# carltonyfakhry/geneticsCRE

Measured on AMD Instinct MI355X. Metric: path_x_permutation_scores_per_sec, higher is better.
Workload: dtype u32

## Files before the change

### geneticscre_amd/api.py

```python
from __future__ import annotations

import ctypes
import functools
import os
from dataclasses import dataclass
from typing import Dict, Optional, Tuple

import numpy as np

from . import build as _build

_LIB = None

GCRE_OK, GCRE_ERR_ASSERT, GCRE_ERR_RANGE, GCRE_ERR_DEVICE, GCRE_ERR_ARG = 0, -1, -2, -3, -4
EXPECTED_ABI = 4


class GcreError(RuntimeError):
    pass


class gcre_result(ctypes.Structure):
    _fields_ = [("n", ctypes.c_int32), ("scores", ctypes.POINTER(ctypes.c_double)),
                ("src", ctypes.POINTER(ctypes.c_int32)), ("trg", ctypes.POINTER(ctypes.c_int32)),
# ... 119 lines not shown
    "gcre_generate_weighted_masks", "gcre_weighted_thresholds", "gcre_weighted_launches",
    "gcre_score_sets_sequential_weighted",
    "gcre_score_sets_prefix_sequential", "gcre_score_sets_dose_sequential", "gcre_seq_prefix_launches",
    "gcre_set_overlap", "gcre_overlap_launches",
    "gcre_clump_sets", "gcre_clump_launches",
    "gcre_set_patient_counts", "gcre_patient_launches",
    "gcre_patient_burden", "gcre_burden_launches",
    "gcre_gene_tally_create", "gcre_join_set_tally", "gcre_process_paths_set_tally", "gcre_gene_tally_read",
    "gcre_gene_tally_free",
    "gcre_exceed_create", "gcre_join_set_exceed", "gcre_process_paths_set_exceed", "gcre_exceed_read",
    "gcre_exceed_reset", "gcre_exceed_free",
    "gcre_exceed_keep_perm_counts", "gcre_exceed_read_perm_counts",
    "gcre_exceed_stepdown", "gcre_stepdown_launches",
    "gcre_hits_create", "gcre_join_set_hits", "gcre_process_paths_set_hits", "gcre_hits_count", "gcre_hits_read",
    "gcre_hits_reset", "gcre_hits_free", "gcre_hits_launches",
    "gcre_test_range_union", "gcre_test_expand",
]


def lib_path() -> str:
    return _build.LIB


def load_library():
    global _LIB
    if _LIB is not None:
        return _LIB
    path = os.environ.get("GCRE_LIB") or _build.build()
    try:
        lib = ctypes.CDLL(path)
    except OSError as e:
# ... 56 lines not shown
    lib.gcre_resolve_count_locs.argtypes = [P, I64, P, P, P, I64, P, P]
    lib.gcre_build_levels.argtypes = [ctypes.c_int32, P, P, P, I64, ctypes.POINTER(gcre_levels)]
    lib.gcre_levels_free.argtypes = [ctypes.POINTER(gcre_levels)]
    lib.gcre_levels_free.restype = None
    lib.gcre_values_table.argtypes = [I, I, P]
    lib.gcre_values_table_exact_order.argtypes = [I, I]
    lib.gcre_rccl_selftest.argtypes = [I, ctypes.c_char_p, ctypes.c_size_t]
    lib.gcre_rccl_collectives.restype = ctypes.c_int64
    lib.gcre_generate_perm_masks.argtypes = [V, ctypes.c_uint64, P, I]
    lib.gcre_mix64.restype = ctypes.c_uint64
    lib.gcre_mix64.argtypes = [ctypes.c_uint64]
    lib.gcre_get_perm_mask.argtypes = [V, I, P]
    if hasattr(lib, "gcre_test_expand"):
        lib.gcre_test_range_union.argtypes = [V, P, I64, P, I64, P, P, P, I64, I, I, I, P, P, P]
        lib.gcre_test_expand.argtypes = [V, P, P, I64, P, I64, I, I, I64, I64, P, P]
    lib.gcre_uids_set_reduced.argtypes = [V, V, P, I64]
    lib.gcre_set_perm_window.argtypes = [V, I, I]
    lib.gcre_plan_perm_window.argtypes = [V, P, I]
    lib.gcre_set_inspect_cache.argtypes = [V, I]
    lib.gcre_drop_inspections.argtypes = [V, I]
    _LIB = lib
    return lib


def _ptr(a: Optional[np.ndarray]):
    return None if a is None else a.ctypes.data_as(ctypes.c_void_p)


_V = _P = ctypes.c_void_p
_I, _I32, _I64 = ctypes.c_int, ctypes.c_int32, ctypes.c_int64
# ... 1149 lines not shown
        piece = np.zeros(1, dtype=np.int32)
        self._check(self._lib.gcre_test_range_union(self._h, _ptr(p1), len(p1), _ptr(pz), len(pz), _ptr(zindex), _ptr(loc), _ptr(cnt),
                                                    len(loc), S, wp, method, _ptr(u), _ptr(bad), _ptr(piece)))
        return u, int(bad[0]), int(piece[0])

    def test_expand(self, path_idx, location, signs, path_length: int, method: int, first: int, count: int):
        path_idx = np.ascontiguousarray(path_idx, dtype=np.int64)
        location = np.ascontiguousarray(location, dtype=np.int64)
        signs = np.ascontiguousarray(signs, dtype=np.int32)
        row0 = np.full(max(count, 1), 0xffffffff, dtype=np.uint32)
        row1 = np.full(max(count, 1), 0xffffffff, dtype=np.uint32)
        self._check(self._lib.gcre_test_expand(self._h, _ptr(path_idx), _ptr(location), len(location), _ptr(signs), len(signs),
                                               int(path_length), int(method), int(first), int(count), _ptr(row0), _ptr(row1)))
        return row0[:count], row1[:count]

    def create_path_set(self, size: int) -> PathSet:
        return PathSet(self, self._lib.gcre_pathset_zeros(self._h, int(size)))

    def load(self, data) -> PathSet:
        d = np.ascontiguousarray(data, dtype=np.int32)
        ncol = d.shape[1] if d.ndim == 2 else 0
        return PathSet(self, self._lib.gcre_pathset_from_dense(self._h, _ptr(d), d.shape[0], ncol, 0))

    def from_words(self, rows) -> PathSet:
        r = np.ascontiguousarray(rows, dtype=np.uint64).reshape(-1, self.vlen)
        return PathSet(self, self._lib.gcre_pathset_from_words(self._h, _ptr(r), r.shape[0]))

    def join(self, uids, paths0: PathSet, paths1: PathSet, paths_res: Optional[PathSet] = None,
             shard: Optional[Tuple[int, int]] = None, d_null_out: int = 0,
             keep: Optional[Tuple[int, int]] = None, keep_mode: int = 1, exchange=None, exchanges: int = 0,
# ... 471 lines not shown
```

### geneticscre_amd/csrc/gcre_host.h

```cpp
#pragma once
#include "../../include/gcre_hip.h"
#include "gcre_kernels.h"
#include "gcre_pipeline.h"

#include <algorithm>
#include <array>
#include <atomic>
#include <chrono>
#include <cmath>
#include <cstdio>
#include <cstdlib>
#include <cstring>
#include <limits>
#include <memory>
#include <mutex>
#include <condition_variable>
#include <string>
#include <unordered_map>
#include <thread>
#include <functional>
#include <deque>
#include <vector>

using namespace gcre;
// ... 243 lines not shown
  int64_t strata_launches = 0;
  int64_t weighted_launches = 0;

  uint64_t* d_case_mask = nullptr;
  uint32_t* d_masks = nullptr;
  float* d_t32 = nullptr;
  double* d_dvt = nullptr;
  double* d_dmax = nullptr;
  double* d_dmaxn = nullptr;
  uint32_t* d_null = nullptr;
  uint32_t* d_mt = nullptr;
  bool mt_stale = false;
  int ieq_batch = 0;
  int ie_quad = 1;
  int ie_flagq = 1;
  int ie_zwide = 0;
  int ie_warm_items = 4;
  int ie_warm_div = 4096;
  int ie_warm_cap_div = 8;
  int exchange_tail = 0;
  int ie_warm_segs = 1024;
  int ie_small_join_tiles = 8;
  int ie_batch = 2;
  uint32_t* d_queue = nullptr;
  uint32_t* d_max_tot = nullptr;
  uint32_t* d_ladder = nullptr;
  uint32_t g00_rows = 0xffffffffu;
  int null_kernel = 0;
  int sparse_waves_per_cu = 32;
  int ie_prune = 1;
// ... 48 lines not shown
};

struct gcre_pathset {
  gcre_ctx* ctx;
  int64_t nrows;
  uint64_t* d_rows;
  uint64_t id = 0;
  mutable uint64_t version = 0;
  mutable gcre_recipe* rec = nullptr;
  mutable uint64_t* d_loff = nullptr;
  mutable uint32_t* d_lidx = nullptr;
  mutable std::vector<uint64_t> h_loff;
  mutable uint32_t max_bits = 0;
  mutable bool max_known = false;
  mutable int one_sided = -1;
  mutable uint32_t* d_planes = nullptr;
  mutable int plane_groups = 0;
  mutable size_t planes_bytes = 0;
  mutable uint64_t planes_epoch = 0;
  mutable bool planes_valid = false;
  mutable int64_t planes_lo = 0, planes_hi = 0;
  mutable bool planes_wanted = false;
};

struct gcre_uids {
  gcre_ctx* ctx;
  int path_length;
  int64_t n_uids;
  int64_t n_signs;
  int64_t total;
// ... 116 lines not shown
```

### geneticscre_amd/csrc/gcre_host.hip

```cpp
#include "gcre_host.h"

namespace {

thread_local std::string g_create_error;

inline bool poison_fresh_planes() {
  static const bool on = std::getenv("GCRE_POISON") != nullptr && std::atoi(std::getenv("GCRE_POISON")) != 0;
  return on;
}
inline void poison_planes(void* p, size_t bytes) {
  if (!poison_fresh_planes() || !p) return;
  (void)hipDeviceSynchronize();
  (void)hipMemset(p, 0x5A, bytes);
  (void)hipDeviceSynchronize();
}

inline size_t tri(size_t t) { return t * (t + 1) / 2; }

template <typename Pred>
void pack_bits_host(const int32_t* data, int64_t nrow, int ncol, bool col_major, uint64_t* out, size_t stride, Pred pred) {
  const int W = (ncol + 63) / 64;
  if (nrow <= 0 || W <= 0) return;
  unsigned T = std::min<unsigned>(16u, std::max(1u, std::thread::hardware_concurrency()));
  if (const char* e = std::getenv("GCRE_PACK_THREADS")) T = (unsigned)std::max(1, std::atoi(e));
// ... 164 lines not shown
        for (size_t k = 1; k < c->plane_pool.size(); k++)
          if (c->plane_pool[k].bytes < c->plane_pool[small].bytes) small = k;
        (void)hipFree(c->plane_pool[small].p);
        c->plane_pool.erase(c->plane_pool.begin() + (long)small);
      }
    } else {
      (void)hipFree(ps->d_planes);
    }
  }
  ps->d_planes = nullptr;
  ps->planes_bytes = 0;
  ps->plane_groups = 0;
  ps->planes_valid = false;
}

void drop_lists(const gcre_pathset* ps) {
  if (ps->d_loff) (void)hipFree(ps->d_loff);
  if (ps->d_lidx) (void)hipFree(ps->d_lidx);
  ps->d_loff = nullptr;
  ps->d_lidx = nullptr;
  ps->h_loff.clear();
  ps->max_bits = 0;
  ps->max_known = false;
  ps->one_sided = -1;
  drop_planes(ps);
}

int ensure_lists(gcre_ctx* c, const gcre_pathset* ps) {
  if (ps->d_loff) return GCRE_OK;
  HostTimer ht("ensure_lists");
  const Geometry& g = c->g;
// ... 28 lines not shown
  ps->h_loff = std::move(off);
  ps->max_bits = longest;
  ps->max_known = true;
  return GCRE_OK;
}

bool one_sided(const gcre_pathset* ps) {
  if (!ps->d_loff || ps->h_loff.size() != (size_t)ps->nrows * 2 + 1) return false;
  if (ps->one_sided < 0) {
    int yes = 1;
    for (int64_t r = 0; r < ps->nrows && yes; r++)
      if (ps->h_loff[(size_t)2 * r + 1] > ps->h_loff[(size_t)2 * r] && ps->h_loff[(size_t)2 * r + 2] > ps->h_loff[(size_t)2 * r + 1]) yes = 0;
    ps->one_sided = yes;
  }
  return ps->one_sided == 1;
}

uint32_t row_max(const gcre_ctx* c, const gcre_pathset* ps) {
  return ps->max_known ? ps->max_bits : (uint32_t)(64 * c->g.Wp);
}

int plane_groups_for(uint32_t max_count) {
  int bits = 1;
  while (bits < 16 && (max_count >> bits) != 0) bits++;
  return std::max(2, (bits + 3) / 4);
}

bool planes_cover(const gcre_ctx* c, const gcre_pathset* ps, int64_t lo, int64_t hi) {
  return ps->d_planes && ps->planes_valid && ps->planes_epoch == c->mask_epoch && (hi <= lo || (ps->planes_lo <= lo && hi <= ps->planes_hi));
}
// ... 1432 lines not shown
    sa.excess = R.hinted ? R.exbuf->p : nullptr;
    sa.range_of = R.hinted ? u.d_range_of : nullptr;
    sa.bad = R.flagblk + kFlagHintBroken;
    sa.ie_bias = 8;
    sa.ie_rule = g.method == 1 ? 1 : 0;
    sa.rowz = C.rowz;
    sa.linfo = C.linfo;
    sa.lover = C.lover;
    sa.slot = C.slot;
    sa.over = C.over;
    sa.over_cap = (uint32_t)std::min<size_t>(C.over_cap - 16, 0xfffffff0u);
    if (rcp && !C.hit) HIP_TRY(c, hipMemcpyAsync(rcp->row0.p + cb, b.row0.p, (size_t)n * 4, hipMemcpyDeviceToDevice, st));
    sa.ov_count = R.flagblk + kFlagOverReserved;
    sa.zoff = (uint32_t)(64 * g.Wp) << 8;
    if (g.method == 2 && one_sided(R.red)) sa.lz_off = R.red->d_loff;
    if (!C.hit) HIP_TRY(c, launch_stats_ie(sa, g.method, st));
    if (rcp && !C.hit)
      HIP_TRY(c, hipMemcpyAsync(rcp->tot.p + (size_t)cb * g.method, b.tot.p, nl * 4, hipMemcpyDeviceToDevice, st));
  } else if (!C.hit) {
    HIP_TRY(c, launch_stats(sa, g.method, st));
  }
  if (!C.hit) {
    HIP_TRY(c, hipEventRecord(e1, st));
    if (R.mode != kInspect) HIP_TRY(c, hipEventRecord(c->ev_insp_main, st));
    R.ev_stats->emplace_back(e0, e1);
    if (ci) {
      ci->inspected = true;
      ci->with_lists = C.use_ie;
      ci->in_recipe = C.use_ie && rcp != nullptr;
    }
// ... 739 lines not shown
  if (const char* e = std::getenv("GCRE_NULL_BLOCKS_PER_CU")) c->null_blocks_per_cu = std::max(1, std::atoi(e));
  if (const char* e = std::getenv("GCRE_NULL_KERNEL"))
    c->null_kernel = !std::strcmp(e, "dense") ? 1 : !std::strcmp(e, "sparse") ? 2 : !std::strcmp(e, "ie") ? 3 : 0;
  if (const char* e = std::getenv("GCRE_IE_PRUNE")) c->ie_prune = std::atoi(e) != 0;
  if (const char* e = std::getenv("GCRE_EXCHANGE_TAIL")) c->exchange_tail = std::min(std::max(std::atoi(e), -1), 64);
  if (const char* e = std::getenv("GCRE_IE_WARM")) c->ie_warm_segs = std::min(std::max(std::atoi(e), 0), 1 << 20);
  if (const char* e = std::getenv("GCRE_IE_WARM_ITEMS")) c->ie_warm_items = std::min(std::max(std::atoi(e), 1), 64);
  if (const char* e = std::getenv("GCRE_IE_WARM_DIV")) c->ie_warm_div = std::min(std::max(std::atoi(e), 1), 1 << 30);
  if (const char* e = std::getenv("GCRE_IE_WARM_CAP_DIV")) c->ie_warm_cap_div = std::min(std::max(std::atoi(e), 1), 1 << 30);
  if (const char* e = std::getenv("GCRE_IE_SJT")) c->ie_small_join_tiles = std::atoi(e);
  if (const char* e = std::getenv("GCRE_IE_BATCH")) c->ie_batch = std::min(std::max(std::atoi(e), 1), 4096);
  if (const char* e = std::getenv("GCRE_IEQ_BATCH")) c->ieq_batch = std::max(0, std::atoi(e));
  if (const char* e = std::getenv("GCRE_IE_QUAD")) c->ie_quad = std::min(std::max(std::atoi(e), 0), 2);
  if (const char* e = std::getenv("GCRE_IE_FLAGQ")) c->ie_flagq = std::atoi(e) != 0;
  if (const char* e = std::getenv("GCRE_IE_ZWIDE")) c->ie_zwide = std::atoi(e) != 0;
  if (const char* e = std::getenv("GCRE_PLANES_OUT_MAX_MB")) c->planes_out_max = (size_t)std::max(0ll, std::atoll(e)) << 20;
  if (const char* e = std::getenv("GCRE_SPARSE_WAVES_PER_CU")) c->sparse_waves_per_cu = std::max(1, std::atoi(e));

  bool ok = hipStreamCreateWithFlags(&c->stream, hipStreamNonBlocking) == hipSuccess;
  ok = ok && hipStreamCreateWithFlags(&c->sel_stream, hipStreamNonBlocking) == hipSuccess;
  ok = ok && hipStreamCreateWithFlags(&c->insp_stream, hipStreamNonBlocking) == hipSuccess;
  ok = ok && hipStreamCreateWithFlags(&c->rec_stream, hipStreamNonBlocking) == hipSuccess;
  ok = ok && hipEventCreateWithFlags(&c->ev_rec_in, hipEventDisableTiming) == hipSuccess;
  ok = ok && hipEventCreateWithFlags(&c->ev_rec_done, hipEventDisableTiming) == hipSuccess;
  if (const char* e = std::getenv("GCRE_REC_STREAM")) c->rec_async = std::atoi(e) != 0;
  ok = ok && hipEventCreateWithFlags(&c->ev_insp_done, hipEventDisableTiming) == hipSuccess;
  ok = ok && hipEventCreateWithFlags(&c->ev_insp_main, hipEventDisableTiming) == hipSuccess;
  ok = ok && hipEventCreateWithFlags(&c->ev_tail, hipEventDisableTiming) == hipSuccess;
  if (const char* e = std::getenv("GCRE_AHEAD")) c->ahead_on = std::atoi(e) != 0;
  ok = ok && hipEventCreateWithFlags(&c->ev_sel, hipEventDisableTiming) == hipSuccess;
// ... 362 lines not shown
  hipError_t e = dpi.upload(path_idx, (size_t)n_uids + 1, st);
  if (e == hipSuccess) e = dloc.upload(location, (size_t)n_uids, st);
  if (e == hipSuccess) e = dsg.upload(signs, (size_t)n_signs, st);
  if (e == hipSuccess) e = d0.reserve((size_t)count);
  if (e == hipSuccess) e = d1.reserve((size_t)count);
  if (e == hipSuccess) e = launch_expand(dpi.p, dloc.p, n_uids, dsg.p, path_length, method, first, count, d0.p, d1.p, st);
  if (e == hipSuccess) e = hipMemcpyAsync(row0, d0.p, (size_t)count * 4, hipMemcpyDeviceToHost, st);
  if (e == hipSuccess) e = hipMemcpyAsync(row1, d1.p, (size_t)count * 4, hipMemcpyDeviceToHost, st);
  if (e == hipSuccess) e = hipStreamSynchronize(st);
  for (void* p : {(void*)dpi.p, (void*)dloc.p, (void*)dsg.p, (void*)d0.p, (void*)d1.p})
    if (p) (void)hipFree(p);
  if (e != hipSuccess) return fail(c, GCRE_ERR_DEVICE, std::string("gcre_test_expand: ") + hipGetErrorString(e));
  return GCRE_OK;
}

gcre_pathset* gcre_pathset_zeros(gcre_ctx* c, int64_t nrows) {
  if (!c) return nullptr;
  (void)hipSetDevice(c->device);
  return new_pathset(c, nrows, true);
}

gcre_pathset* gcre_pathset_from_dense(gcre_ctx* c, const int32_t* data, int64_t nrow, int ncol, int col_major) {
  if (!c) return nullptr;
  (void)hipSetDevice(c->device);
  if (nrow < 0 || ncol < 0 || (!data && nrow > 0 && ncol > 0)) {
    fail(c, GCRE_ERR_ARG, "bad dense matrix");
    return nullptr;
  }
  if (ncol > c->g.W * 64) {
    fail(c, GCRE_ERR_RANGE, "assertion: more data columns than mask bits");
// ... 256 lines not shown
```

### geneticscre_amd/csrc/gcre_inspect.hip

```cpp
#include "gcre_ie_common.h"

namespace gcre {

__device__ __forceinline__ u64 ie_score_key(double s) {
  if (!(s > -__builtin_inf())) return 0;
  const u64 b = (u64)__double_as_longlong(s);
  return (b >> 63) ? ~b : (b | 0x8000000000000000ull);
}

__device__ __forceinline__ u32 row_scan_add(u32 v) {
  u32 s = v;
  s += (u32)__builtin_amdgcn_update_dpp(0, (int)v, 0x111, 0xf, 0xf, true);
  s += (u32)__builtin_amdgcn_update_dpp(0, (int)v, 0x112, 0xf, 0xf, true);
  s += (u32)__builtin_amdgcn_update_dpp(0, (int)v, 0x113, 0xf, 0xf, true);
  s += (u32)__builtin_amdgcn_update_dpp(0, (int)s, 0x114, 0xf, 0xe, true);
  s += (u32)__builtin_amdgcn_update_dpp(0, (int)s, 0x118, 0xf, 0xc, true);
  return s;
}
__device__ __forceinline__ u32 row_last(u32 v, int lane) {
  return (u32)__builtin_amdgcn_ds_bpermute(((lane | 15) << 2), (int)v);
}
__device__ __forceinline__ u32 row_total(u32 v, int lane) { return row_last(row_scan_add(v), lane); }

struct OverChunk {
// ... 230 lines not shown
                              int64_t npieces, const int32_t* cut, int64_t ncut, int S, int Wp, int method, uint64_t* excess,
                              uint32_t* bad, hipStream_t stream) {
  if (npieces == 0) return hipSuccess;
  if (ncut) {
    const i64 zb = (ncut * (S >> 1) + 255) / 256;
    hipLaunchKernelGGL(k_range_zero, dim3((unsigned)(zb < 4096 ? zb : 4096)), dim3(256), 0, stream, cut, ncut, S, excess);
  }
  const i64 blocks = (npieces * ((S + 31) >> 5) + 3) / 4;
  const i64 grid = blocks < kRangeUnionMaxBlocks ? blocks : kRangeUnionMaxBlocks;
  trace_launch("k_range_union", blocks, grid);
  hipLaunchKernelGGL(k_range_union, dim3((unsigned)grid), dim3(256), 0, stream, p1, pz, zindex, pieces, npieces, S, Wp, method,
                     excess, bad);
  return hipGetLastError();
}

constexpr int kStatsWaves = 4;
template <int NL>
__global__ __launch_bounds__(256) __attribute__((amdgpu_waves_per_eu(NL <= 3 ? kStatsWaves : 2))) void k_stats_ie2(const StatsArgs a) {
  typedef u64 __attribute__((ext_vector_type(2))) u64x2;
  constexpr u32 kNoRange = 0xffffffffu;
  __shared__ u32 slot_lds[4][64 * 8];
  __shared__ u32 out_lds[4][8][64];
  __shared__ u32 pair_lds[4][4][3][32 * NL];
  const int lane = threadIdx.x & 63;
  const int wv = __builtin_amdgcn_readfirstlane(threadIdx.x >> 6);
  const int sl = lane & 15, grp = lane >> 4;
  const u32 gsh = (u32)grp * 16u, ltm = (1u << sl) - 1u;
  u32 (*pairs)[32 * NL] = pair_lds[wv][grp];
  __shared__ u32 meta_lds[4][3][64];
  u32 (*meta)[64] = meta_lds[wv];
  const i64 wave = (i64)blockIdx.x * 4 + wv;
  const i64 nwaves = (i64)gridDim.x * 4;
// ... 18 lines not shown
    meta[0][lane] = r0v;
    meta[1][lane] = zv & 0x7fffffffu;
    meta[2][lane] = rngv;
    __builtin_amdgcn_wave_barrier();
    {
      const u32x4 pad = {a.zoff, a.zoff, a.zoff, a.zoff};
      ((u32x4*)slots)[lane * 2] = pad;
      ((u32x4*)slots)[lane * 2 + 1] = pad;
    }
    double score_prev = 0.0;
    int pl_prev = -1;
    u64 xw[NL][2], zw[NL][2];
#pragma unroll
    for (int it = 0; it < NL; it++) xw[it][0] = xw[it][1] = zw[it][0] = zw[it][1] = 0ull;
    u32 n_rz = 0u, n_rng = kNoRange, n_r0 = 0xffffffffu;
    auto fetch_rows = [&](int it4n) {
      const int pln = it4n * 4 + grp;
      const u32 r0n = meta[0][pln];
      n_rz = meta[1][pln];
      n_rng = meta[2][pln];
      const bool new_x = r0n != n_r0;
      n_r0 = r0n;
      const u64* xn = a.p0 + (size_t)r0n * a.S;
      const u64* zn = a.pz + (size_t)n_rz * a.S;
#pragma unroll
      for (int it = 0; it < NL; it++) {
        const int k = it * 32 + 2 * sl;
        if (k < Wp) {
          if (new_x) {
            const u64x2 v = *(const u64x2*)(xn + k);
            xw[it][0] = v.x; xw[it][1] = v.y;
          }
          const u64x2 v = *(const u64x2*)(zn + k);
          zw[it][0] = v.x; zw[it][1] = v.y;
        }
      }
    };
    fetch_rows(0);
    for (int it4 = 0; it4 < 16; it4++) {
      const int pl = it4 * 4 + grp;
      const bool active = base + pl < a.count;
      if (__builtin_amdgcn_ballot_w64(active) == 0ull) break;
      const u32 rz = n_rz, rng = n_rng;
      const u64* uu = (rng != kNoRange) ? a.excess + (size_t)rng * a.S : nullptr;
      u64* out = (a.res && active) ? a.res + (size_t)(a.first + base + pl) * a.S : nullptr;
      u32 cc = 0u, dv = 0u;
      u64 stray = 0;
#pragma unroll
      for (int it = 0; it < NL; it++) {
        const int k = it * 32 + 2 * sl;
        u64x2 uv = {0, 0};
        if (k < Wp && uu) uv = *(const u64x2*)(uu + k);
        const u64x2 cmv = *(const u64x2*)(cm_lds + k);
        const u64 cme[2] = {cmv.x, cmv.y};
#pragma unroll
        for (int e = 0; e < 2; e++) {
          const u64 xk = xw[it][e], zk = zw[it][e], uk = e ? uv.y : uv.x;
          stray |= uk & ~xk;
          const u64 j = xk | zk;
          cc += (u32)__popcll(j & cme[e]) | ((u32)__popcll(j) << 16);
          dv += (u32)__popcll(zk & ~xk) | ((u32)__popcll(zk) << 16);
        }
        if (out && k < Wp) *(u64x2*)(out + k) = u64x2{xw[it][0] | zw[it][0], xw[it][1] | zw[it][1]};
      }
      if (stray) my_bad = true;
      const u32 c = row_total(cc, lane), d = row_total(dv, lane);
      const u32 inc = c & 0xffffu, tot = c >> 16, inm = tot - inc;
      const u32 dl = d & 0xffffu, ov = (d >> 16) - dl;
      const u32 mode = a.ie_rule ? ((ov <= 8u || ov < dl) ? 1u : 0u) : ((a.ie_bias >= 0 && ov + (u32)a.ie_bias < dl) ? 1u : 0u);
      const u32 len = mode ? ov : dl;
      const u32 len8 = max(8u, (len + 7u) & ~7u);
      u32 npair = 0u;
#pragma unroll
      for (int it = 0; it < NL; it++) {
#pragma unroll
        for (int e = 0; e < 2; e++) {
          const u64 w = mode ? (zw[it][e] & xw[it][e]) : (zw[it][e] & ~xw[it][e]);
          const bool nz = active && w != 0;
          const u64 bal = __builtin_amdgcn_ballot_w64(nz);
          if (bal == 0ull) continue;
          const u32 m = (u32)(bal >> gsh) & 0xffffu;
          const u32 at = npair + (u32)__builtin_popcount(m & ltm);
          if (nz) {
            pairs[0][at] = (u32)w;
            pairs[1][at] = (u32)(w >> 32);
            pairs[2][at] = (u32)(it * 32 + 2 * sl + e);
          }
          npair += (u32)__builtin_popcount(m);
        }
      }
      fetch_rows(it4 < 15 ? it4 + 1 : 15);
      double score = 0.0;
      if (active && sl == 0) {
        my_modes += mode;
        my_max_tot = max(my_max_tot, tot);
        my_max_len = max(my_max_len, len8);
        score = a.dvt[(size_t)sp_diag_offset(tot) + inc];
      }
      const u32 need = (active && len8 > 8u) ? len8 - 8u : 0u;
      const u32 ovb = chunk.take(need, grp, lane, a.ov_count);
      const bool ov_ok = active && len8 > 8u && (u64)ovb + (len8 - 8u) <= (u64)a.over_cap;
      u32* over = a.over + ovb;
      __builtin_amdgcn_wave_barrier();
      {
        const u32 npmax = max(max(rdlane(npair, 0), rdlane(npair, 16)), max(rdlane(npair, 32), rdlane(npair, 48)));
// ... 510 lines not shown

using StatsKernel = void (*)(StatsArgs);
static hipError_t launch_staged(const StatsKernel (&kernel)[5], const char* name, i64 per_wave, const StatsArgs& a,
                                hipStream_t stream) {
  const i64 nb = (a.count + per_wave - 1) / per_wave;
  const i64 blocks = (nb + kInspectBlockWaves - 1) / kInspectBlockWaves;
  const dim3 grid((unsigned)(blocks < kInspectMaxBlocks ? blocks : kInspectMaxBlocks)), block(64 * kInspectBlockWaves);
  const int nl = (a.Wp + 31) / 32;
  trace_launch(name, blocks, grid.x);
  hipLaunchKernelGGL(kernel[nl <= 1 ? 0 : nl - 1], grid, block, 0, stream, a);
  return hipGetLastError();
}

hipError_t launch_stats_ie(const StatsArgs& a, int method, hipStream_t stream) {
  if (a.count == 0) return hipSuccess;
  static const StatsKernel ie2[5] = {k_stats_ie2<1>, k_stats_ie2<2>, k_stats_ie2<3>, k_stats_ie2<4>, k_stats_ie2<5>};
  static const StatsKernel ie2h[5] = {k_stats_ie2h<1>, k_stats_ie2h<2>, k_stats_ie2h<3>, k_stats_ie2h<4>, k_stats_ie2h<5>};
  static const StatsKernel ie2s[5] = {k_stats_ie2s<1>, k_stats_ie2s<2>, k_stats_ie2s<3>, k_stats_ie2s<4>, k_stats_ie2s<5>};
  if (a.Wp <= 160) {
    if (method == 1) return launch_staged(ie2, "k_stats_ie2", 64, a, stream);
    if (a.lz_off) return launch_staged(ie2h, "k_stats_ie2h", 64, a, stream);
    return launch_staged(ie2s, "k_stats_ie2s", 32, a, stream);
  }
  const i64 blocks = (a.count + kStatsIeBlockPaths - 1) / kStatsIeBlockPaths;
  const dim3 grid((unsigned)(blocks < kInspectMaxBlocks ? blocks : kInspectMaxBlocks)), block(64 * kInspectBlockWaves);
  trace_launch("k_stats_ie<M>", blocks, grid.x);
  if (method == 1) hipLaunchKernelGGL(k_stats_ie<1>, grid, block, 0, stream, a);
  else hipLaunchKernelGGL(k_stats_ie<2>, grid, block, 0, stream, a);
  return hipGetLastError();
}

}
```

### geneticscre_amd/csrc/gcre_kernels.h

```cpp
#pragma once

#include <hip/hip_runtime.h>
#include <stdint.h>
#include <stdio.h>

namespace gcre {

extern bool g_launch_trace __attribute__((visibility("hidden")));
inline void trace_launch(const char* kernel, long long want, long long got) {
  if (g_launch_trace) fprintf(stderr, "launch %s want=%lld got=%lld\n", kernel, want, got);
}

struct Geometry {
  int method;
  int n;
  int n_cases;
  int W;
  int Wp;
  int S;
  int K;
  int Kpad;
  int TD;
};

// ... 185 lines not shown
  const int32_t* zindex;
  uint32_t* rowz;
  uint32_t* bad;
  int ie_bias;
  int ie_rule;
  const uint64_t* excess;
  const int32_t* range_of;
  uint32_t* linfo;
  uint32_t* lover;
  uint32_t* slot;
  uint32_t* over;
  uint32_t over_cap;
  uint32_t* ov_count;
  uint32_t zoff;
  const uint64_t* lz_off;
  int64_t first;
  int64_t count;
  int S;
  int Wp;
};
constexpr uint32_t kOverChunk = 2048;
constexpr int kInspectBlockWaves = 4;
constexpr int kInspectMaxBlocks = 256 * 16;
constexpr int kStatsIeBlockPaths = 4 * kInspectBlockWaves;
hipError_t launch_stats(const StatsArgs& a, int method, hipStream_t stream);
hipError_t launch_stats_ie(const StatsArgs& a, int method, hipStream_t stream);
constexpr int kRangePieceRows = 16;
struct RangePiece {
  int64_t first;
  int32_t range;
  int32_t rows;
};
hipError_t launch_range_union(const uint64_t* p1, const uint64_t* pz, const int32_t* zindex, const RangePiece* pieces,
                              int64_t npieces, const int32_t* cut, int64_t ncut, int S, int Wp, int method, uint64_t* excess,
                              uint32_t* bad, hipStream_t stream);

hipError_t launch_hist(const uint64_t* key, int64_t count, int shift, uint64_t prefix, uint32_t* hist256,
                       hipStream_t stream);
struct SelectState {
  uint64_t prefix;
  int64_t need;
// ... 625 lines not shown
```

### include/gcre_hip.h

```cpp
#ifndef GCRE_HIP_H
#define GCRE_HIP_H

#include <stddef.h>
#include <stdint.h>

#ifdef __cplusplus
extern "C" {
#endif

#define GCRE_ABI_VERSION 4

typedef enum {
  GCRE_OK = 0,
  GCRE_ERR_ASSERT = -1,
  GCRE_ERR_RANGE = -2,
  GCRE_ERR_DEVICE = -3,
  GCRE_ERR_ARG = -4
} gcre_status;

typedef struct gcre_ctx gcre_ctx;
typedef struct gcre_pathset gcre_pathset;

typedef struct {
  int32_t n;
// ... 154 lines not shown
int gcre_values_table(int n_cases, int n_ctrls, double* out);
int gcre_values_table_exact_order(int n_cases, int n_ctrls);

int gcre_generate_perm_masks(gcre_ctx* ctx, uint64_t seed, const int32_t* stratum, int n_strata);
uint64_t gcre_mix64(uint64_t z);
int gcre_set_perm_window(gcre_ctx* ctx, int k0, int k1);
int gcre_plan_perm_window(gcre_ctx* ctx, const int64_t* set_rows, int n_sets);
int gcre_set_inspect_cache(gcre_ctx* ctx, int on);
int gcre_drop_inspections(gcre_ctx* ctx, int release_memory);
int gcre_get_perm_mask(gcre_ctx* ctx, int r, uint64_t* out);
int gcre_test_range_union(gcre_ctx* ctx, const uint64_t* p1, int64_t n1, const uint64_t* pz, int64_t nz, const int32_t* zindex,
                          const int64_t* loc, const int32_t* cnt, int64_t n_ranges, int S, int Wp, int method, uint64_t* u_out,
                          uint32_t* bad_out, int32_t* piece_rows_out);
int gcre_test_expand(gcre_ctx* ctx, const int64_t* path_idx, const int64_t* location, int64_t n_uids, const int32_t* signs,
                     int64_t n_signs, int path_length, int method, int64_t first, int64_t count, uint32_t* row0, uint32_t* row1);


typedef struct {
  int32_t pop;
  int32_t cases;
  int32_t k_pos;
  int32_t k_neg;
} gcre_dp_stratum;

typedef struct {
  int32_t method;
  int32_t n_cases, n_ctrls;
  int32_t n_paths;
  const int32_t* path_len;
  const int32_t* path_rows;
// ... 228 lines not shown
```

Baseline: 10660 billion.

## Precompute per-row popcounts and use inclusion-exclusion for overlap stats in inspector

Adds a one-time kernel that stores, for each reduced-set row, its total and case popcounts, cached on the pathset with an event for cross-stream use. A new CNT variant of the method-1 stats kernel computes union counts as count(x)+count(z)-count(x&z). It gets the overlap count from the compacted pairs it already builds, computes x counts only when the x row changes, and builds the delta list only for paths that need it. This removes per-path popcount passes over the union and delta words, at the cost of extra memory, a prelaunch kernel and more branching. A test entry point for the inspector is also added.

```diff
diff --git a/geneticscre_amd/api.py b/geneticscre_amd/api.py
--- a/geneticscre_amd/api.py
+++ b/geneticscre_amd/api.py
@@ -157,7 +157,7 @@
     "gcre_exceed_stepdown", "gcre_stepdown_launches",
     "gcre_hits_create", "gcre_join_set_hits", "gcre_process_paths_set_hits", "gcre_hits_count", "gcre_hits_read",
     "gcre_hits_reset", "gcre_hits_free", "gcre_hits_launches",
-    "gcre_test_range_union", "gcre_test_expand",
+    "gcre_test_range_union", "gcre_test_expand", "gcre_test_inspect",
 ]
 
 
@@ -244,6 +244,8 @@
     if hasattr(lib, "gcre_test_expand"):
         lib.gcre_test_range_union.argtypes = [V, P, I64, P, I64, P, P, P, I64, I, I, I, P, P, P]
         lib.gcre_test_expand.argtypes = [V, P, P, I64, P, I64, I, I, I64, I64, P, P]
+    if hasattr(lib, "gcre_test_inspect"):
+        lib.gcre_test_inspect.argtypes = [V, V, V, P, P, I64, P, I64, P, P, I64, I64, P, P, P, P, P, P, P, I64, P, P]
     lib.gcre_uids_set_reduced.argtypes = [V, V, P, I64]
     lib.gcre_set_perm_window.argtypes = [V, I, I]
     lib.gcre_plan_perm_window.argtypes = [V, P, I]
@@ -1423,6 +1425,41 @@
                                                int(path_length), int(method), int(first), int(count), _ptr(row0), _ptr(row1)))
         return row0[:count], row1[:count]
 
+    def test_inspect(self, p0: PathSet, red: PathSet, row0, row1, zindex=None, excess=None, range_of=None,
+                     over_entries: Optional[int] = None, ent_stride: Optional[int] = None, keep_rows: bool = False) -> dict:
+        row0 = np.ascontiguousarray(row0, dtype=np.uint32)
+        row1 = np.ascontiguousarray(row1, dtype=np.uint32)
+        n = len(row0)
+        assert len(row1) == n
+        if zindex is not None:
+            zindex = np.ascontiguousarray(zindex, dtype=np.int32)
+        if excess is not None:
+            excess = np.ascontiguousarray(excess, dtype=np.uint64).reshape(-1, self.vlen)
+            range_of = np.ascontiguousarray(range_of, dtype=np.int32)
+            assert len(range_of) == p0.size
+        stride = int(ent_stride) if ent_stride is not None else 64 * self.vlen + 8
+        over = int(over_entries) if over_entries is not None else n * stride
+        out = {k: np.zeros(max(n, 1), dtype=np.uint32) for k in ("tot", "cases", "ctrls", "rowz", "linfo")}
+        out["key"] = np.zeros(max(n, 1), dtype=np.uint64)
+        entries = np.zeros((max(n, 1), stride), dtype=np.uint32)
+        rows = np.zeros((max(n, 1), self.vlen), dtype=np.uint64) if keep_rows else None
+        flags = np.zeros(8, dtype=np.uint32)
+        self._check(self._lib.gcre_test_inspect(
+            self._h, p0._h, red._h, _ptr(row0), _ptr(row1), n, _ptr(zindex) if zindex is not None else None,
+            len(zindex) if zindex is not None else 0, _ptr(excess) if excess is not None else None,
+            _ptr(range_of) if excess is not None else None, len(excess) if excess is not None else 0, over,
+            _ptr(out["tot"]), _ptr(out["cases"]), _ptr(out["ctrls"]), _ptr(out["rowz"]), _ptr(out["linfo"]), _ptr(out["key"]),
+            _ptr(entries), stride, _ptr(rows) if keep_rows else None, _ptr(flags)))
+        out = {k: v[:n] for k, v in out.items()}
+        len8 = (out["linfo"] & 0x0ffffff8).astype(np.int64)
+        pad = (out["linfo"] >> 28).astype(np.int64)
+        out["lists"] = [entries[i, :len8[i] - pad[i]] for i in range(n)]
+        out["padding"] = [entries[i, len8[i] - pad[i]:len8[i]] for i in range(n)]
+        out["flags"] = flags
+        if keep_rows:
+            out["rows"] = rows[:n]
+        return out
+
     def create_path_set(self, size: int) -> PathSet:
         return PathSet(self, self._lib.gcre_pathset_zeros(self._h, int(size)))
 
diff --git a/geneticscre_amd/csrc/gcre_host.h b/geneticscre_amd/csrc/gcre_host.h
--- a/geneticscre_amd/csrc/gcre_host.h
+++ b/geneticscre_amd/csrc/gcre_host.h
@@ -281,6 +281,7 @@
   int ieq_batch = 0;
   int ie_quad = 1;
   int ie_flagq = 1;
+  int stats_ie_counts = 1;
   int ie_zwide = 0;
   int ie_warm_items = 4;
   int ie_warm_div = 4096;
@@ -359,6 +360,9 @@
   mutable uint32_t max_bits = 0;
   mutable bool max_known = false;
   mutable int one_sided = -1;
+  mutable uint32_t* d_counts = nullptr;
+  mutable hipStream_t counts_on = nullptr;
+  mutable hipEvent_t counts_ev = nullptr;
   mutable uint32_t* d_planes = nullptr;
   mutable int plane_groups = 0;
   mutable size_t planes_bytes = 0;
diff --git a/geneticscre_amd/csrc/gcre_host.hip b/geneticscre_amd/csrc/gcre_host.hip
--- a/geneticscre_amd/csrc/gcre_host.hip
+++ b/geneticscre_amd/csrc/gcre_host.hip
@@ -202,7 +202,10 @@
   ps->planes_valid = false;
 }
 
+void drop_row_counts(const gcre_pathset* ps);
+
 void drop_lists(const gcre_pathset* ps) {
+  drop_row_counts(ps);
   if (ps->d_loff) (void)hipFree(ps->d_loff);
   if (ps->d_lidx) (void)hipFree(ps->d_lidx);
   ps->d_loff = nullptr;
@@ -261,6 +264,35 @@
     ps->one_sided = yes;
   }
   return ps->one_sided == 1;
+}
+
+void drop_row_counts(const gcre_pathset* ps) {
+  if (ps->d_counts) (void)hipFree(ps->d_counts);
+  if (ps->counts_ev) (void)hipEventDestroy(ps->counts_ev);
+  ps->d_counts = nullptr;
+  ps->counts_ev = nullptr;
+  ps->counts_on = nullptr;
+}
+
+int row_counts_for(gcre_ctx* c, const gcre_pathset* ps, int64_t paths, hipStream_t st, const uint32_t** out) {
+  *out = nullptr;
+  const Geometry& g = c->g;
+  if (!c->stats_ie_counts || g.method != 1 || g.Wp > 160 || ps->nrows <= 0 || ps->nrows > paths) return GCRE_OK;
+  if (!ps->d_counts) {
+    HIP_TRY(c, hipMalloc((void**)&ps->d_counts, (size_t)ps->nrows * 4));
+    hipError_t e = launch_row_counts(ps->d_rows, ps->nrows, g.Wp, c->d_case_mask, ps->d_counts, st);
+    if (e == hipSuccess) e = hipEventCreateWithFlags(&ps->counts_ev, hipEventDisableTiming);
+    if (e == hipSuccess) e = hipEventRecord(ps->counts_ev, st);
+    if (e != hipSuccess) {
+      drop_row_counts(ps);
+      return fail(c, GCRE_ERR_DEVICE, std::string("row counts: ") + hipGetErrorString(e));
+    }
+    ps->counts_on = st;
+  } else if (ps->counts_on != st) {
+    HIP_TRY(c, hipStreamWaitEvent(st, ps->counts_ev, 0));
+  }
+  *out = ps->d_counts;
+  return GCRE_OK;
 }
 
 uint32_t row_max(const gcre_ctx* c, const gcre_pathset* ps) {
@@ -1723,6 +1755,8 @@
     sa.ov_count = R.flagblk + kFlagOverReserved;
     sa.zoff = (uint32_t)(64 * g.Wp) << 8;
     if (g.method == 2 && one_sided(R.red)) sa.lz_off = R.red->d_loff;
+    if (!C.hit)
+      if (int rc = row_counts_for(c, R.red, R.P, st, &sa.z_counts)) return rc;
     if (!C.hit) HIP_TRY(c, launch_stats_ie(sa, g.method, st));
     if (rcp && !C.hit)
       HIP_TRY(c, hipMemcpyAsync(rcp->tot.p + (size_t)cb * g.method, b.tot.p, nl * 4, hipMemcpyDeviceToDevice, st));
@@ -2492,6 +2526,7 @@
   if (const char* e = std::getenv("GCRE_IE_QUAD")) c->ie_quad = std::min(std::max(std::atoi(e), 0), 2);
   if (const char* e = std::getenv("GCRE_IE_FLAGQ")) c->ie_flagq = std::atoi(e) != 0;
   if (const char* e = std::getenv("GCRE_IE_ZWIDE")) c->ie_zwide = std::atoi(e) != 0;
+  if (const char* e = std::getenv("GCRE_STATS_IE_COUNTS")) c->stats_ie_counts = std::atoi(e) != 0;
   if (const char* e = std::getenv("GCRE_PLANES_OUT_MAX_MB")) c->planes_out_max = (size_t)std::max(0ll, std::atoll(e)) << 20;
   if (const char* e = std::getenv("GCRE_SPARSE_WAVES_PER_CU")) c->sparse_waves_per_cu = std::max(1, std::atoi(e));
 
@@ -2884,6 +2919,122 @@
   return GCRE_OK;
 }
 
+int gcre_test_inspect(gcre_ctx* c, const gcre_pathset* p0, const gcre_pathset* red, const uint32_t* row0, const uint32_t* row1,
+                      int64_t count, const int32_t* zindex, int64_t n_zindex, const uint64_t* excess, const int32_t* range_of,
+                      int64_t n_ranges, int64_t over_entries, uint32_t* tot, uint32_t* cases, uint32_t* ctrls, uint32_t* rowz,
+                      uint32_t* linfo, uint64_t* key, uint32_t* entries, int64_t ent_stride, uint64_t* res_out, uint32_t* flags) {
+  if (!c) return GCRE_ERR_ARG;
+  const Geometry& g = c->g;
+  if (!p0 || !red || p0->ctx != c || red->ctx != c || !row0 || !row1 || count <= 0 || count > (1 << 24) || over_entries < 0 ||
+      !tot || !cases || !ctrls || !rowz || !linfo || !key || !entries || ent_stride < 8 || !flags || (zindex && n_zindex <= 0) ||
+      ((excess != nullptr) != (range_of != nullptr)) || (excess && (!zindex || n_ranges <= 0)))
+    return fail(c, GCRE_ERR_ARG, "gcre_test_inspect: bad arguments");
+  if (g.method != 1 || g.Wp > 160) return fail(c, GCRE_ERR_ARG, "gcre_test_inspect: the block-staged method-1 inspector only");
+  if (!c->d_dvt) return fail(c, GCRE_ERR_ARG, "gcre_test_inspect: no value table");
+  for (int64_t i = 0; i < count; i++) {
+    if ((int64_t)row0[i] >= p0->nrows) return fail(c, GCRE_ERR_RANGE, "gcre_test_inspect: paths0 row out of range");
+    if ((row1[i] >> 31) || (int64_t)row1[i] >= (zindex ? n_zindex : red->nrows))
+      return fail(c, GCRE_ERR_RANGE, "gcre_test_inspect: paths1 row out of range");
+    if (zindex && (zindex[row1[i]] < 0 || (int64_t)zindex[row1[i]] >= red->nrows))
+      return fail(c, GCRE_ERR_RANGE, "gcre_test_inspect: reduced row out of range");
+    if (range_of && (range_of[row0[i]] < 0 || (int64_t)range_of[row0[i]] >= n_ranges))
+      return fail(c, GCRE_ERR_RANGE, "gcre_test_inspect: range out of range");
+  }
+  (void)hipSetDevice(c->device);
+  hipStream_t st = c->stream;
+  const size_t n = (size_t)count;
+  const size_t blocks = (n + kStatsIeBlockPaths - 1) / kStatsIeBlockPaths;
+  const size_t over_cap = (size_t)over_entries + (std::min<size_t>((size_t)kInspectMaxBlocks, blocks) * kInspectBlockWaves + 2) * kOverChunk + 16;
+  DevBuf<uint32_t> d0, d1, dtot, dcases, dctrls, drowz, dlinfo, dlover, dslot, dover, dflags;
+  DevBuf<int32_t> dzi, drng;
+  DevBuf<uint64_t> dkey, dex, dres;
+  std::vector<uint32_t> lover(n), slot(n * 8), over;
+  hipError_t e = d0.upload(row0, n, st);
+  if (e == hipSuccess) e = d1.upload(row1, n, st);
+  if (e == hipSuccess && zindex) e = dzi.upload(zindex, (size_t)n_zindex, st);
+  if (e == hipSuccess && excess) e = dex.reserve((size_t)n_ranges * g.S);
+  if (e == hipSuccess && excess) e = hipMemsetAsync(dex.p, 0, (size_t)n_ranges * g.S * 8, st);
+  if (e == hipSuccess && excess)
+    e = hipMemcpy2DAsync(dex.p, (size_t)g.S * 8, excess, (size_t)g.W * 8, (size_t)g.W * 8, (size_t)n_ranges, hipMemcpyHostToDevice, st);
+  if (e == hipSuccess && excess) e = drng.upload(range_of, (size_t)p0->nrows, st);
+  for (DevBuf<uint32_t>* b : {&dtot, &dcases, &dctrls, &drowz, &dlinfo, &dlover})
+    if (e == hipSuccess) e = b->reserve(n);
+  if (e == hipSuccess) e = dkey.reserve(n);
+  if (e == hipSuccess) e = dslot.reserve(n * 8);
+  if (e == hipSuccess) e = dover.reserve(over_cap);
+  if (e == hipSuccess) e = dflags.reserve(kFlagWords);
+  if (e == hipSuccess && res_out) e = dres.reserve(n * g.S);
+  if (e == hipSuccess) e = hipMemsetAsync(dflags.p, 0, kFlagWords * 4, st);
+  StatsArgs sa{};
+  int rc = GCRE_OK;
+  if (e == hipSuccess) {
+    sa.p0 = p0->d_rows;
+    sa.p1 = red->d_rows;
+    sa.pz = red->d_rows;
+    sa.row0 = d0.p;
+    sa.row1 = d1.p;
+    sa.case_mask = c->d_case_mask;
+    sa.dvt = c->d_dvt;
+    sa.key = dkey.p;
+    sa.tot = dtot.p;
+    sa.cases = dcases.p;
+    sa.ctrls = dctrls.p;
+    sa.res = res_out ? dres.p : nullptr;
+    sa.max_tot = dflags.p;
+    sa.zindex = zindex ? dzi.p : nullptr;
+    sa.excess = excess ? dex.p : nullptr;
+    sa.range_of = excess ? drng.p : nullptr;
+    sa.rowz = drowz.p;
+    sa.bad = dflags.p + kFlagHintBroken;
+    sa.ie_bias = 8;
+    sa.ie_rule = 1;
+    sa.linfo = dlinfo.p;
+    sa.lover = dlover.p;
+    sa.slot = dslot.p;
+    sa.over = dover.p;
+    sa.over_cap = (uint32_t)std::min<size_t>(over_cap - 16, 0xfffffff0u);
+    sa.ov_count = dflags.p + kFlagOverReserved;
+    sa.zoff = (uint32_t)(64 * g.Wp) << 8;
+    sa.first = 0;
+    sa.count = count;
+    sa.S = g.S;
+    sa.Wp = g.Wp;
+    rc = row_counts_for(c, red, count, st, &sa.z_counts);
+  }
+  if (rc == GCRE_OK) {
+    if (e == hipSuccess) e = launch_stats_ie(sa, 1, st);
+    for (auto pr : {std::make_pair(tot, dtot.p), std::make_pair(cases, dcases.p), std::make_pair(ctrls, dctrls.p),
+                    std::make_pair(rowz, drowz.p), std::make_pair(linfo, dlinfo.p), std::make_pair(lover.data(), dlover.p)})
+      if (e == hipSuccess) e = hipMemcpyAsync(pr.first, pr.second, n * 4, hipMemcpyDeviceToHost, st);
+    if (e == hipSuccess) e = hipMemcpyAsync(key, dkey.p, n * 8, hipMemcpyDeviceToHost, st);
+    if (e == hipSuccess) e = hipMemcpyAsync(slot.data(), dslot.p, n * 32, hipMemcpyDeviceToHost, st);
+    if (e == hipSuccess) e = hipMemcpyAsync(flags, dflags.p, kFlagWords * 4, hipMemcpyDeviceToHost, st);
+    if (e == hipSuccess && res_out)
+      e = hipMemcpy2DAsync(res_out, (size_t)g.W * 8, dres.p, (size_t)g.S * 8, (size_t)g.W * 8, n, hipMemcpyDeviceToHost, st);
+    if (e == hipSuccess) e = hipStreamSynchronize(st);
+    if (e == hipSuccess && flags[kFlagOverReserved] > sa.over_cap) rc = fail(c, GCRE_ERR_RANGE, "gcre_test_inspect: the lists need more overflow entries than given");
+    if (e == hipSuccess && rc == GCRE_OK && flags[kFlagOverReserved]) {
+      over.resize(flags[kFlagOverReserved]);
+      e = hipMemcpy(over.data(), dover.p, over.size() * 4, hipMemcpyDeviceToHost);
+    }
+  }
+  for (void* p : {(void*)d0.p, (void*)d1.p, (void*)dtot.p, (void*)dcases.p, (void*)dctrls.p, (void*)drowz.p, (void*)dlinfo.p,
+                  (void*)dlover.p, (void*)dslot.p, (void*)dover.p, (void*)dflags.p, (void*)dzi.p, (void*)drng.p, (void*)dkey.p,
+                  (void*)dex.p, (void*)dres.p})
+    if (p) (void)hipFree(p);
+  if (rc != GCRE_OK) return rc;
+  if (e != hipSuccess) return fail(c, GCRE_ERR_DEVICE, std::string("gcre_test_inspect: ") + hipGetErrorString(e));
+  for (size_t i = 0; i < n; i++) {
+    const uint32_t len8 = linfo_len(linfo[i]);
+    if ((int64_t)len8 > ent_stride) return fail(c, GCRE_ERR_RANGE, "gcre_test_inspect: a list is longer than the room per path");
+    if (len8 > 8 && (size_t)lover[i] + (len8 - 8) > over.size()) return fail(c, GCRE_ERR_DEVICE, "gcre_test_inspect: a list's overflow part lies outside the area");
+    uint32_t* dst = entries + i * (size_t)ent_stride;
+    std::copy(slot.begin() + (long)(i * 8), slot.begin() + (long)(i * 8 + 8), dst);
+    if (len8 > 8) std::copy(over.begin() + lover[i], over.begin() + lover[i] + (len8 - 8), dst + 8);
+  }
+  return GCRE_OK;
+}
+
 gcre_pathset* gcre_pathset_zeros(gcre_ctx* c, int64_t nrows) {
   if (!c) return nullptr;
   (void)hipSetDevice(c->device);
diff --git a/geneticscre_amd/csrc/gcre_inspect.hip b/geneticscre_amd/csrc/gcre_inspect.hip
--- a/geneticscre_amd/csrc/gcre_inspect.hip
+++ b/geneticscre_amd/csrc/gcre_inspect.hip
@@ -268,8 +268,49 @@
   return hipGetLastError();
 }
 
+constexpr int kRowCountsMaxBlocks = 1024;
+__global__ __launch_bounds__(256) void k_row_counts(const u64* rows, i64 nrows, int Wp, const u64* case_mask, u32* counts) {
+  typedef u64 __attribute__((ext_vector_type(2))) u64x2;
+  const int lane = threadIdx.x & 63, sl = lane & 15;
+  const i64 ngroups = (i64)gridDim.x * 16;
+  for (i64 r0 = (i64)blockIdx.x * 16 + (threadIdx.x >> 6) * 4; r0 < nrows; r0 += ngroups) {
+    const i64 r = r0 + (lane >> 4);
+    const bool valid = r < nrows;
+    u64x2 v[5];
+#pragma unroll
+    for (int it = 0; it < 5; it++) {
+      const int k = it * 32 + 2 * sl;
+      v[it] = u64x2{0ull, 0ull};
+      if (valid && k < Wp) v[it] = *(const u64x2*)(rows + (size_t)r * Wp + k);
+    }
+    u32 c = 0u;
+#pragma unroll
+    for (int it = 0; it < 5; it++) {
+      const int k = it * 32 + 2 * sl;
+      if (k < Wp) {
+        const u64x2 cm = *(const u64x2*)(case_mask + k);
+        c += (u32)__popcll(v[it].x) + (u32)__popcll(v[it].y) +
+             (((u32)__popcll(v[it].x & cm.x) + (u32)__popcll(v[it].y & cm.y)) << 16);
+      }
+    }
+    c = row_total(c, lane);
+    if (valid && sl == 0) counts[r] = c;
+  }
+}
+
+hipError_t launch_row_counts(const uint64_t* rows, int64_t nrows, int Wp, const uint64_t* case_mask, uint32_t* counts,
+                             hipStream_t stream) {
+  if (nrows == 0) return hipSuccess;
+  if (Wp > 160 || (Wp & 3)) return hipErrorInvalidValue;
+  const i64 blocks = (nrows + 15) / 16;
+  const i64 grid = blocks < kRowCountsMaxBlocks ? blocks : kRowCountsMaxBlocks;
+  trace_launch("k_row_counts", blocks, grid);
+  hipLaunchKernelGGL(k_row_counts, dim3((unsigned)grid), dim3(256), 0, stream, rows, nrows, Wp, case_mask, counts);
+  return hipGetLastError();
+}
+
 constexpr int kStatsWaves = 4;
-template <int NL>
+template <int NL, bool CNT>
 __global__ __launch_bounds__(256) __attribute__((amdgpu_waves_per_eu(NL <= 3 ? kStatsWaves : 2))) void k_stats_ie2(const StatsArgs a) {
   typedef u64 __attribute__((ext_vector_type(2))) u64x2;
   constexpr u32 kNoRange = 0xffffffffu;
@@ -318,6 +359,8 @@
 #pragma unroll
     for (int it = 0; it < NL; it++) xw[it][0] = xw[it][1] = zw[it][0] = zw[it][1] = 0ull;
     u32 n_rz = 0u, n_rng = kNoRange, n_r0 = 0xffffffffu;
+    u32 n_zc = 0u, x_cnt = 0u;
+    bool n_newx = false;
     auto fetch_rows = [&](int it4n) {
       const int pln = it4n * 4 + grp;
       const u32 r0n = meta[0][pln];
@@ -325,6 +368,10 @@
       n_rng = meta[2][pln];
       const bool new_x = r0n != n_r0;
       n_r0 = r0n;
+      if constexpr (CNT) {
+        n_newx = new_x;
+        n_zc = a.z_counts[n_rz];
+      }
       const u64* xn = a.p0 + (size_t)r0n * a.S;
       const u64* zn = a.pz + (size_t)n_rz * a.S;
 #pragma unroll
@@ -348,51 +395,141 @@
       const u32 rz = n_rz, rng = n_rng;
       const u64* uu = (rng != kNoRange) ? a.excess + (size_t)rng * a.S : nullptr;
       u64* out = (a.res && active) ? a.res + (size_t)(a.first + base + pl) * a.S : nullptr;
-      u32 cc = 0u, dv = 0u;
-      u64 stray = 0;
-#pragma unroll
-      for (int it = 0; it < NL; it++) {
-        const int k = it * 32 + 2 * sl;
-        u64x2 uv = {0, 0};
-        if (k < Wp && uu) uv = *(const u64x2*)(uu + k);
-        const u64x2 cmv = *(const u64x2*)(cm_lds + k);
-        const u64 cme[2] = {cmv.x, cmv.y};
-#pragma unroll
-        for (int e = 0; e < 2; e++) {
-          const u64 xk = xw[it][e], zk = zw[it][e], uk = e ? uv.y : uv.x;
-          stray |= uk & ~xk;
-          const u64 j = xk | zk;
-          cc += (u32)__popcll(j & cme[e]) | ((u32)__popcll(j) << 16);
-          dv += (u32)__popcll(zk & ~xk) | ((u32)__popcll(zk) << 16);
-        }
-        if (out && k < Wp) *(u64x2*)(out + k) = u64x2{xw[it][0] | zw[it][0], xw[it][1] | zw[it][1]};
-      }
-      if (stray) my_bad = true;
-      const u32 c = row_total(cc, lane), d = row_total(dv, lane);
-      const u32 inc = c & 0xffffu, tot = c >> 16, inm = tot - inc;
-      const u32 dl = d & 0xffffu, ov = (d >> 16) - dl;
-      const u32 mode = a.ie_rule ? ((ov <= 8u || ov < dl) ? 1u : 0u) : ((a.ie_bias >= 0 && ov + (u32)a.ie_bias < dl) ? 1u : 0u);
-      const u32 len = mode ? ov : dl;
+      u32 inc, tot, inm, mode, len, npair = 0u;
+      if constexpr (CNT) {
+        if (__builtin_amdgcn_ballot_w64(rng != kNoRange) != 0ull) {
+          u64 stray = 0;
+#pragma unroll
+          for (int it = 0; it < NL; it++) {
+            const int k = it * 32 + 2 * sl;
+            u64x2 uv = {0, 0};
+            if (k < Wp && uu) uv = *(const u64x2*)(uu + k);
+            stray |= (uv.x & ~xw[it][0]) | (uv.y & ~xw[it][1]);
+          }
+          if (stray) my_bad = true;
+        }
+        if (out) {
+#pragma unroll
+          for (int it = 0; it < NL; it++) {
+            const int k = it * 32 + 2 * sl;
+            if (k < Wp) *(u64x2*)(out + k) = u64x2{xw[it][0] | zw[it][0], xw[it][1] | zw[it][1]};
+          }
+        }
+        if (n_newx) {
+          u32 xc = 0u;
+#pragma unroll
+          for (int it = 0; it < NL; it++) {
+            const u64x2 cmv = *(const u64x2*)(cm_lds + it * 32 + 2 * sl);
+            xc += (u32)__popcll(xw[it][0]) + (u32)__popcll(xw[it][1]) +
+                  (((u32)__popcll(xw[it][0] & cmv.x) + (u32)__popcll(xw[it][1] & cmv.y)) << 16);
+          }
+          x_cnt = row_total(xc, lane);
+        }
+        const u32 zc = n_zc;
+#pragma unroll
+        for (int it = 0; it < NL; it++) {
+#pragma unroll
+          for (int e = 0; e < 2; e++) {
+            const u64 w = zw[it][e] & xw[it][e];
+            const bool nz = active && w != 0;
+            const u64 bal = __builtin_amdgcn_ballot_w64(nz);
+            if (bal == 0ull) continue;
+            const u32 m = (u32)(bal >> gsh) & 0xffffu;
+            const u32 at = npair + (u32)__builtin_popcount(m & ltm);
+            if (nz) {
+              pairs[0][at] = (u32)w;
+              pairs[1][at] = (u32)(w >> 32);
+              pairs[2][at] = (u32)(it * 32 + 2 * sl + e);
+            }
+            npair += (u32)__builtin_popcount(m);
+          }
+        }
+        __builtin_amdgcn_wave_barrier();
+        u32 ovc = 0u;
+        {
+          const u32 npmax = max(max(rdlane(npair, 0), rdlane(npair, 16)), max(rdlane(npair, 32), rdlane(npair, 48)));
+          for (u32 p0 = 0u; p0 < npmax; p0 += 16u) {
+            const u32 pi = p0 + (u32)sl;
+            const bool has = pi < npair;
+            const u64 w = has ? ((u64)pairs[1][pi] << 32) | (u64)pairs[0][pi] : 0ull;
+            const u32 k = has ? pairs[2][pi] : 0u;
+            ovc += (u32)__popcll(w) | ((u32)__popcll(w & cm_lds[k]) << 16);
+          }
+          if (npmax != 0u) ovc = row_total(ovc, lane);
+        }
+        const u32 c = x_cnt + zc - ovc;
+        tot = c & 0xffffu, inc = c >> 16, inm = tot - inc;
+        const u32 ov = ovc & 0xffffu, dl = (zc & 0xffffu) - ov;
+        mode = a.ie_rule ? ((ov <= 8u || ov < dl) ? 1u : 0u) : ((a.ie_bias >= 0 && ov + (u32)a.ie_bias < dl) ? 1u : 0u);
+        len = mode ? ov : dl;
+        const bool delta = active && mode == 0u;
+        if (__builtin_amdgcn_ballot_w64(delta) != 0ull) {
+          if (delta) npair = 0u;
+#pragma unroll
+          for (int it = 0; it < NL; it++) {
+#pragma unroll
+            for (int e = 0; e < 2; e++) {
+              const u64 w = zw[it][e] & ~xw[it][e];
+              const bool nz = delta && w != 0;
+              const u64 bal = __builtin_amdgcn_ballot_w64(nz);
+              if (bal == 0ull) continue;
+              const u32 m = (u32)(bal >> gsh) & 0xffffu;
+              const u32 at = npair + (u32)__builtin_popcount(m & ltm);
+              if (nz) {
+                pairs[0][at] = (u32)w;
+                pairs[1][at] = (u32)(w >> 32);
+                pairs[2][at] = (u32)(it * 32 + 2 * sl + e);
+              }
+              npair += (u32)__builtin_popcount(m);
+            }
+          }
+        }
+      } else {
+        u32 cc = 0u, dv = 0u;
+        u64 stray = 0;
+#pragma unroll
+        for (int it = 0; it < NL; it++) {
+          const int k = it * 32 + 2 * sl;
+          u64x2 uv = {0, 0};
+          if (k < Wp && uu) uv = *(const u64x2*)(uu + k);
+          const u64x2 cmv = *(const u64x2*)(cm_lds + k);
+          const u64 cme[2] = {cmv.x, cmv.y};
+#pragma unroll
+          for (int e = 0; e < 2; e++) {
+            const u64 xk = xw[it][e], zk = zw[it][e], uk = e ? uv.y : uv.x;
+            stray |= uk & ~xk;
+            const u64 j = xk | zk;
+            cc += (u32)__popcll(j & cme[e]) | ((u32)__popcll(j) << 16);
+            dv += (u32)__popcll(zk & ~xk) | ((u32)__popcll(zk) << 16);
+          }
+          if (out && k < Wp) *(u64x2*)(out + k) = u64x2{xw[it][0] | zw[it][0], xw[it][1] | zw[it][1]};
+        }
+        if (stray) my_bad = true;
+        const u32 c = row_total(cc, lane), d = row_total(dv, lane);
+        inc = c & 0xffffu, tot = c >> 16, inm = tot - inc;
+        const u32 dl = d & 0xffffu, ov = (d >> 16) - dl;
+        mode = a.ie_rule ? ((ov <= 8u || ov < dl) ? 1u : 0u) : ((a.ie_bias >= 0 && ov + (u32)a.ie_bias < dl) ? 1u : 0u);
+        len = mode ? ov : dl;
+#pragma unroll
+        for (int it = 0; it < NL; it++) {
+#pragma unroll
+          for (int e = 0; e < 2; e++) {
+            const u64 w = mode ? (zw[it][e] & xw[it][e]) : (zw[it][e] & ~xw[it][e]);
+            const bool nz = active && w != 0;
+            const u64 bal = __builtin_amdgcn_ballot_w64(nz);
+            if (bal == 0ull) continue;
+            const u32 m = (u32)(bal >> gsh) & 0xffffu;
+            const u32 at = npair + (u32)__builtin_popcount(m & ltm);
+            if (nz) {
+              pairs[0][at] = (u32)w;
+              pairs[1][at] = (u32)(w >> 32);
+              pairs[2][at] = (u32)(it * 32 + 2 * sl + e);
+            }
+            npair += (u32)__builtin_popcount(m);
+          }
+        }
+      }
       const u32 len8 = max(8u, (len + 7u) & ~7u);
-      u32 npair = 0u;
-#pragma unroll
-      for (int it = 0; it < NL; it++) {
-#pragma unroll
-        for (int e = 0; e < 2; e++) {
-          const u64 w = mode ? (zw[it][e] & xw[it][e]) : (zw[it][e] & ~xw[it][e]);
-          const bool nz = active && w != 0;
-          const u64 bal = __builtin_amdgcn_ballot_w64(nz);
-          if (bal == 0ull) continue;
-          const u32 m = (u32)(bal >> gsh) & 0xffffu;
-          const u32 at = npair + (u32)__builtin_popcount(m & ltm);
-          if (nz) {
-            pairs[0][at] = (u32)w;
-            pairs[1][at] = (u32)(w >> 32);
-            pairs[2][at] = (u32)(it * 32 + 2 * sl + e);
-          }
-          npair += (u32)__builtin_popcount(m);
-        }
-      }
       fetch_rows(it4 < 15 ? it4 + 1 : 15);
       double score = 0.0;
       if (active && sl == 0) {
@@ -933,10 +1070,14 @@
 
 hipError_t launch_stats_ie(const StatsArgs& a, int method, hipStream_t stream) {
   if (a.count == 0) return hipSuccess;
-  static const StatsKernel ie2[5] = {k_stats_ie2<1>, k_stats_ie2<2>, k_stats_ie2<3>, k_stats_ie2<4>, k_stats_ie2<5>};
+  static const StatsKernel ie2[5] = {k_stats_ie2<1, false>, k_stats_ie2<2, false>, k_stats_ie2<3, false>, k_stats_ie2<4, false>,
+                                     k_stats_ie2<5, false>};
+  static const StatsKernel ie2c[5] = {k_stats_ie2<1, true>, k_stats_ie2<2, true>, k_stats_ie2<3, true>, k_stats_ie2<4, true>,
+                                      k_stats_ie2<5, true>};
   static const StatsKernel ie2h[5] = {k_stats_ie2h<1>, k_stats_ie2h<2>, k_stats_ie2h<3>, k_stats_ie2h<4>, k_stats_ie2h<5>};
   static const StatsKernel ie2s[5] = {k_stats_ie2s<1>, k_stats_ie2s<2>, k_stats_ie2s<3>, k_stats_ie2s<4>, k_stats_ie2s<5>};
   if (a.Wp <= 160) {
+    if (method == 1 && a.z_counts) return launch_staged(ie2c, "k_stats_ie2", 64, a, stream);
     if (method == 1) return launch_staged(ie2, "k_stats_ie2", 64, a, stream);
     if (a.lz_off) return launch_staged(ie2h, "k_stats_ie2h", 64, a, stream);
     return launch_staged(ie2s, "k_stats_ie2s", 32, a, stream);
diff --git a/geneticscre_amd/csrc/gcre_kernels.h b/geneticscre_amd/csrc/gcre_kernels.h
--- a/geneticscre_amd/csrc/gcre_kernels.h
+++ b/geneticscre_amd/csrc/gcre_kernels.h
@@ -223,6 +223,7 @@
   uint32_t* ov_count;
   uint32_t zoff;
   const uint64_t* lz_off;
+  const uint32_t* z_counts;
   int64_t first;
   int64_t count;
   int S;
@@ -234,6 +235,8 @@
 constexpr int kStatsIeBlockPaths = 4 * kInspectBlockWaves;
 hipError_t launch_stats(const StatsArgs& a, int method, hipStream_t stream);
 hipError_t launch_stats_ie(const StatsArgs& a, int method, hipStream_t stream);
+hipError_t launch_row_counts(const uint64_t* rows, int64_t nrows, int Wp, const uint64_t* case_mask, uint32_t* counts,
+                             hipStream_t stream);
 constexpr int kRangePieceRows = 16;
 struct RangePiece {
   int64_t first;
diff --git a/include/gcre_hip.h b/include/gcre_hip.h
--- a/include/gcre_hip.h
+++ b/include/gcre_hip.h
@@ -192,6 +192,10 @@
                           uint32_t* bad_out, int32_t* piece_rows_out);
 int gcre_test_expand(gcre_ctx* ctx, const int64_t* path_idx, const int64_t* location, int64_t n_uids, const int32_t* signs,
                      int64_t n_signs, int path_length, int method, int64_t first, int64_t count, uint32_t* row0, uint32_t* row1);
+int gcre_test_inspect(gcre_ctx* ctx, const gcre_pathset* p0, const gcre_pathset* red, const uint32_t* row0, const uint32_t* row1,
+                      int64_t count, const int32_t* zindex, int64_t n_zindex, const uint64_t* excess, const int32_t* range_of,
+                      int64_t n_ranges, int64_t over_entries, uint32_t* tot, uint32_t* cases, uint32_t* ctrls, uint32_t* rowz,
+                      uint32_t* linfo, uint64_t* key, uint32_t* entries, int64_t ent_stride, uint64_t* res_out, uint32_t* flags);
 
 
 typedef struct {
```

After: 10840 billion, median of 6. 1.7% higher.
